# EavnJeong/IEF-VAD

Hardware: AMD Instinct MI355X
Metric: snippets/sec at [B,T=256,d=768] (higher is better)
Workload: dtype f32 emulated: exact 3-term bf16 split of both fp32 operands, 6 bf16 MFMA products, fp32 accumulate

## Files before the change

### ief-vad_amd/csrc/gemm_split.h

```cpp
#pragma once
#include "gemm_bf16.h"

#ifndef GS_EXP_NODMA
#define GS_EXP_NODMA 0
#endif
#ifndef GS_EXP_NOSPLIT
#define GS_EXP_NOSPLIT 0
#endif
#ifndef GS_EXP_NOBAR
#define GS_EXP_NOBAR 0
#endif
#ifndef GS_PN
#define GS_PN 6
#endif
#define GS_BM 128
#define GS_BK 32
#define GS_A_SLOT (GS_BM * 32)
#define GS_BN_OF(NA) ((NA) == 4 ? 256 : 128)
#define GS_LDS_BYTES_OF(NA) ((2 * GS_A_SLOT + 2 * 3 * GS_BN_OF(NA) * 16) * 4)
#define GS_BN GS_BN_OF(4)
#define GS_LDS_BYTES GS_LDS_BYTES_OF(4)

typedef float f32x2 __attribute__((ext_vector_type(2)));
typedef __bf16 bf16x2 __attribute__((ext_vector_type(2)));
typedef unsigned u32x4 __attribute__((ext_vector_type(4)));
typedef _Float16 f16x2 __attribute__((ext_vector_type(2)));
typedef _Float16 f16x8 __attribute__((ext_vector_type(8)));

__device__ __forceinline__ unsigned cvt_pk_bf16(float lo, float hi) {
    return __builtin_bit_cast(unsigned, __builtin_convertvector(f32x2{lo, hi}, bf16x2));
}

struct Split4 {
    f32x4 r;
    __device__ __forceinline__ void plane(unsigned& d0, unsigned& d1, bool peel) {
        d0 = cvt_pk_bf16(r[0], r[1]);
        d1 = cvt_pk_bf16(r[2], r[3]);
        if (peel) {
            r[0] -= __builtin_bit_cast(float, d0 << 16);
            r[1] -= __builtin_bit_cast(float, d0 & 0xffff0000u);
            r[2] -= __builtin_bit_cast(float, d1 << 16);
            r[3] -= __builtin_bit_cast(float, d1 & 0xffff0000u);
        }
    }
    __device__ __forceinline__ void plane_f16(unsigned& d0, unsigned& d1, bool peel) {
        const f16x2 a = __builtin_convertvector(f32x2{r[0], r[1]}, f16x2), b = __builtin_convertvector(f32x2{r[2], r[3]}, f16x2);
        d0 = __builtin_bit_cast(unsigned, a);
        d1 = __builtin_bit_cast(unsigned, b);
        if (peel) {
            const f32x2 fa = __builtin_convertvector(a, f32x2), fb = __builtin_convertvector(b, f32x2);
            r[0] -= fa[0]; r[1] -= fa[1]; r[2] -= fb[0]; r[3] -= fb[1];
        }
    }
};

__global__ __launch_bounds__(256) void iefvad_split_planes_kernel(const float* __restrict__ src, bf16_t* __restrict__ planes, size_t n) {
    const size_t stride = (size_t)gridDim.x * blockDim.x * 4;
    for (size_t i = ((size_t)blockIdx.x * blockDim.x + threadIdx.x) * 4; i < n; i += stride) {
        Split4 s;
        s.r = *(const f32x4*)(src + i);
#pragma unroll
        for (int p = 0; p < 3; ++p) {
            unsigned d0, d1;
            s.plane(d0, d1, p < 2);
            *(uint2*)(planes + (size_t)p * n + i) = make_uint2(d0, d1);
        }
    }
}

#define SPLIT_MANY_MAX 32
struct SplitManyArgs {
    const float* src[SPLIT_MANY_MAX];
    bf16_t* dst[SPLIT_MANY_MAX];
    unsigned n[SPLIT_MANY_MAX];
    int rows[SPLIT_MANY_MAX];
    int count;
};
__global__ __launch_bounds__(256) void iefvad_split_planes_many_kernel(SplitManyArgs a) {
    const int z = blockIdx.y;
    const float* __restrict__ src = a.src[z];
    bf16_t* __restrict__ planes = a.dst[z];
    const size_t n = a.n[z];
    const int n_out = a.rows[z];
    if (n_out == 0) {
// ... 220 lines not shown
                _Pragma("unroll") for (int p = 0; p < NP; ++p) wn[p] = *(const u32x4*)(Wv + p * W_PLANE + ((B) + 1) * 16 * 16); \
                if (GS_NAREAD(B) == 1) vn0 = a_half((B) + 1);                                                   \
                if (GS_NAREAD(B) == 2) { vn0 = a_half((B) + 1); vn1 = a_half((B) + 2); }                        \
            }                                                                                                   \
            if constexpr (!F16) {                                                                               \
                mfma_row(B, NP - 1, w[0]);                                                           \
                mfma_row(B, 0, w[NP - 1]);                                                           \
                mfma_row(B, 1, w[1]);                                                                \
            }                                                                                                   \
            mfma_row(B, 1, w[0]);                                                                    \
            mfma_row(B, 0, w[1]);                                                                    \
            mfma_row(B, 0, w[0]);                                                                    \
            if (!GS_EXP_NOSPLIT) {                                                                              \
                if (GS_NSPLIT(B) >= 1) split_half(B, v0);                                                       \
                if (GS_NSPLIT(B) == 2) split_half((B) + 1, v1);                                                 \
            }                                                                                                   \
            if ((B) == 7) {                                                                                     \
                _Pragma("unroll") for (int a = 0; a < NA; ++a)                                                  \
                    _Pragma("unroll") for (int p = 0; p < NP; ++p) ap[a][p] = an[a][p];                         \
            }                                                                                                   \
            _Pragma("unroll") for (int d = 0; d < GS_NDMA(B); ++d) dma(GS_NDMA(B) * (B) + d);                   \
            if (GS_NREAD(B) > 0) __builtin_amdgcn_sched_group_barrier(0x100, GS_NREAD(B) > 0 ? GS_NREAD(B) : 1, 0); \
            GS_SLOT(B, 0) GS_SLOT(B, 1) GS_SLOT(B, 2) GS_SLOT(B, 3) GS_SLOT(B, 4) GS_SLOT(B, 5)                 \
            GS_SLOT(B, 6) GS_SLOT(B, 7) GS_SLOT(B, 8) GS_SLOT(B, 9) GS_SLOT(B, 10) GS_SLOT(B, 11)               \
            GS_SLOT(B, 12) GS_SLOT(B, 13) GS_SLOT(B, 14) GS_SLOT(B, 15) GS_SLOT(B, 16) GS_SLOT(B, 17)           \
            GS_SLOT(B, 18) GS_SLOT(B, 19) GS_SLOT(B, 20) GS_SLOT(B, 21) GS_SLOT(B, 22) GS_SLOT(B, 23)           \
            GS_FENCE();                                                                                         \
            if ((B) < 7) {                                                                                      \
                _Pragma("unroll") for (int p = 0; p < NP; ++p) w[p] = wn[p];                                    \
                if (GS_NAREAD(B) >= 1) v0 = vn0;                                                                \
                if (GS_NAREAD(B) == 2) v1 = vn1;                                                                \
            }                                                                                                   \
        }
        GS_STEP(0) GS_STEP(1) GS_STEP(2) GS_STEP(3) GS_STEP(4) GS_STEP(5) GS_STEP(6) GS_STEP(7)
#undef GS_STEP
#undef GS_SLOT
#undef GS_VSLOT
#undef GS_NVALU
#undef GS_NDMA
#undef GS_NREAD
#undef GS_NAREAD
#undef GS_NSPLIT
        GS_DIAG_STAMP(0)
        asm volatile("s_waitcnt vmcnt(0)" ::: "memory");
        asm volatile("s_waitcnt lgkmcnt(0)" ::: "memory");
        GS_DIAG_STAMP(1)
        if (!GS_EXP_NOBAR) GB2_BARRIER();
        GS_DIAG_STAMP(2)
    }
#ifdef GB2_CLOCK_DIAG
    if (threadIdx.x == 0 && P.C2) {
        unsigned long long* dg = (unsigned long long*)P.C2 + 2 * (blockIdx.x + gridDim.x * blockIdx.z);
        dg[0] = __builtin_amdgcn_s_memtime() - dg_c0;
        dg[1] = __builtin_amdgcn_s_memrealtime() - dg_r0;
        unsigned long long* dx = (unsigned long long*)P.C2 + 2 * gridDim.x * gridDim.z + 3 * (blockIdx.x + gridDim.x * blockIdx.z);
        dx[0] = dg_acc[0]; dx[1] = dg_acc[1]; dx[2] = dg_acc[2];
    }
    const unsigned long long dg_loop_end = __builtin_amdgcn_s_memtime();
#endif
#undef GS_PIPE
#undef GS_FENCE
#undef GLDS16
    f32x16 unused[NA / 2][4];
    gemm_wave_epilogue<true, NA / 2, !F16>(args, P, smem, m0, n0, wrow0, wcol0, unused, acc16, cscale, F16 ? P.amaxC : nullptr);
#ifdef GB2_CLOCK_DIAG
    if (threadIdx.x == 0 && P.C2) {
        unsigned long long* dy = (unsigned long long*)P.C2 + 5 * gridDim.x * gridDim.z + 2 * (blockIdx.x + gridDim.x * blockIdx.z);
        dy[0] = dg_c0 - dg_entry;
        dy[1] = __builtin_amdgcn_s_memtime() - dg_loop_end;
    }
#endif
}

__global__ __launch_bounds__(256, 1) void iefvad_gemm_split_kernel(GemmBArgs args) {
    extern __shared__ __attribute__((aligned(16))) float smem[];
    gemm_split_body<4>(args, smem);
}

__global__ __launch_bounds__(256, 2) void iefvad_gemm_split_n128_kernel(GemmBArgs args) {
    extern __shared__ __attribute__((aligned(16))) float smem[];
    gemm_split_body<2>(args, smem);
}

__global__ __launch_bounds__(256, 2) void iefvad_gemm_split_f16_n128_kernel(GemmBArgs args) {
    extern __shared__ __attribute__((aligned(16))) float smem[];
    gemm_split_body<2, true>(args, smem);
}

#ifdef GS_EXPERIMENT_F16
__global__ __launch_bounds__(256, 1) void iefvad_gemm_split_f16_kernel(GemmBArgs args) {
    extern __shared__ __attribute__((aligned(16))) float smem[];
    gemm_split_body<4, true>(args, smem);
}
#endif

__global__ __launch_bounds__(256) void iefvad_split_planes_f16_kernel(const float* __restrict__ src, _Float16* __restrict__ planes,
                                                                      size_t n, const float* __restrict__ amax) {
    const float scale = __builtin_ldexpf(1.0f, 13 - amax_exponent(amax_read(amax)));
    const size_t stride = (size_t)gridDim.x * blockDim.x * 4;
    for (size_t i = ((size_t)blockIdx.x * blockDim.x + threadIdx.x) * 4; i < n; i += stride) {
        Split4 s;
        s.r = *(const f32x4*)(src + i) * scale;
#pragma unroll
        for (int p = 0; p < 2; ++p) {
            unsigned d0, d1;
            s.plane_f16(d0, d1, p < 1);
            *(uint2*)(planes + (size_t)p * n + i) = make_uint2(d0, d1);
        }
    }
}
```

### ief-vad_amd/csrc/iefvad.hip

```cpp
#include "../../include/iefvad.h"

#include <hip/hip_runtime.h>
#include <math.h>
#include <stdarg.h>
#include <stdio.h>
#include <stdlib.h>
#include <string.h>

#include <algorithm>
#include <exception>
#include <new>
#include <thread>
#include <vector>

#include "attention_f32.h"
#include "attention_bf16.h"
#include "attention_pbf16.h"
#include "attention_split.h"
#include "common.h"
#include "gather.h"
#include "gemm_f32.h"
#include "gemm_bf16.h"
#include "gemm_split.h"
#include "rowops.h"
// ... 131 lines not shown
            return fail("%s: kernels are built for D=768, T=256, H=8, or D=512, T=256, H=8 in the f32 arithmetic (got D=%d T=%d H=%d)", who,
                        cfg->embed_dim, cfg->seq_len, cfg->num_heads);
        return fail("iefvad_create: kernels are built for D=768, T=256, H=8 (got D=%d T=%d H=%d)",
                    cfg->embed_dim, cfg->seq_len, cfg->num_heads);
    }
    if (cfg->num_layers < 1 || cfg->num_layers > IEFVAD_MAX_LAYERS)
        return fail("%s: num_layers %d outside 1..%d", who, cfg->num_layers, IEFVAD_MAX_LAYERS);
    if (cfg->num_steps < 0 || cfg->num_steps > IEFVAD_MAX_STEPS)
        return fail("%s: num_steps %d outside 0..%d", who, cfg->num_steps, IEFVAD_MAX_STEPS);
    if (cfg->noise_model != IEFVAD_NOISE_GAUSSIAN && cfg->noise_model != IEFVAD_NOISE_STUDENT_T)
        return fail("Unsupported noise_model. Choose 'Gaussian' or 'StudentT'.");
    if (cfg->compute != IEFVAD_COMPUTE_F32 && cfg->compute != IEFVAD_COMPUTE_BF16 && cfg->compute != IEFVAD_COMPUTE_BF16X6 &&
        cfg->compute != IEFVAD_COMPUTE_FP16X3)
        return fail("%s: unknown compute mode %d", who, cfg->compute);
    if (cfg->noise_model == IEFVAD_NOISE_STUDENT_T && !(cfg->nu != 0.f))
        return fail("%s: nu must be non-zero for StudentT", who);
    int ndev = 0;
    HIP_TRY(hipGetDeviceCount(&ndev));
    if (ndev <= 0) return fail("%s: no HIP device", who);
    iefvad_handle* h = new (std::nothrow) iefvad_handle();
    if (!h) return fail("%s: out of host memory", who);
    memset(h, 0, sizeof(*h));
    h->cfg = *cfg;
    h->D = d512 ? IEF_D512 : IEF_D;
    h->DH = h->D / IEF_H;
    {
        const char* v = getenv("IEFVAD_ROWBLOCK_OFF");
        const int off = v ? atoi(v) : 0;
        h->no_inproj_chain = off & 1; h->no_ln_fusion = off & 2; h->no_heads_fusion = off & 4; h->no_chain = off & 8;
    }
    { const char* v = getenv("IEFVAD_ROWBLOCK_MIN_WGS"); h->rowblock_min_wgs = (v && atoi(v) > 0) ? atoi(v) : 128; }
    { const char* v = getenv("IEFVAD_CHAIN_MIN_BLOCKS"); h->chain_min_blocks = (v && atoi(v) > 0) ? atoi(v) : 4; }
    { const char* v = getenv("IEFVAD_PERSIST"); h->persist = !(v && v[0] == '0'); }
    { const char* v = getenv("IEFVAD_DENSE_ENCODER"); h->dense_encoder = v && v[0] == '1'; }
    { const char* v = getenv("IEFVAD_TRAIN_ATTN"); h->train_attn_unfused = v && v[0] == 'u'; }
    { const char* v = getenv("IEFVAD_HOSTPIPE_TRACE"); h->hostpipe_trace = v && v[0] == '1'; }
    hipError_t e = hipGetDevice(&h->device);
    if (e == hipSuccess)
        e = hipFuncSetAttribute((const void*)iefvad_gemm_bf16_kernel, hipFuncAttributeMaxDynamicSharedMemorySize,
                                GB2_LDS_BYTES);
    if (e == hipSuccess)
        e = hipFuncSetAttribute((const void*)iefvad_gemm_bf16_pipe_kernel, hipFuncAttributeMaxDynamicSharedMemorySize,
                                GB2_LDS_BYTES);
    if (e == hipSuccess)
        e = hipFuncSetAttribute((const void*)iefvad_gemm_bf16_w256_kernel, hipFuncAttributeMaxDynamicSharedMemorySize,
                                GB3_LDS_BYTES);
    if (e == hipSuccess)
        e = hipFuncSetAttribute((const void*)iefvad_refine_chain_bf16_kernel, hipFuncAttributeMaxDynamicSharedMemorySize,
                                RC_LDS_BYTES);
    if (e == hipSuccess)
        e = hipFuncSetAttribute((const void*)iefvad_outproj_ln_chain_bf16_kernel, hipFuncAttributeMaxDynamicSharedMemorySize,
                                OC_LDS_BYTES);
    if (e == hipSuccess)
        e = hipFuncSetAttribute((const void*)iefvad_outproj_ln_pchain_bf16_kernel<true, true>, hipFuncAttributeMaxDynamicSharedMemorySize,
                                OP_LDS_BYTES);
    if (e == hipSuccess)
        e = hipFuncSetAttribute((const void*)iefvad_outproj_ln_pchain_bf16_kernel<true, false>, hipFuncAttributeMaxDynamicSharedMemorySize,
                                OP_LDS_BYTES);
    if (e == hipSuccess)
        e = hipFuncSetAttribute((const void*)iefvad_outproj_ln_pchain_bf16_kernel<false, true>, hipFuncAttributeMaxDynamicSharedMemorySize,
                                OP_LDS_BYTES);
    if (e == hipSuccess)
        e = hipFuncSetAttribute((const void*)iefvad_heads_pchain_bf16_kernel, hipFuncAttributeMaxDynamicSharedMemorySize,
                                HP_LDS_BYTES);
    if (e == hipSuccess)
        e = hipFuncSetAttribute((const void*)iefvad_gemm_split_tn256_kernel, hipFuncAttributeMaxDynamicSharedMemorySize, TN_LDS_BYTES_OF(4));
    if (e == hipSuccess)
        e = hipFuncSetAttribute((const void*)iefvad_attention_pbf16_kernel, hipFuncAttributeMaxDynamicSharedMemorySize, APB_LDS_BYTES);
    if (e == hipSuccess)
        e = hipFuncSetAttribute((const void*)iefvad_attention_pbf16_rows_kernel, hipFuncAttributeMaxDynamicSharedMemorySize, APB_LDS_BYTES);
    if (e == hipSuccess) {
        hipDeviceProp_t prop;
        e = hipGetDeviceProperties(&prop, h->device);
        h->num_cus = e == hipSuccess ? prop.multiProcessorCount : 256;
        g_num_cus = h->num_cus;
    }
    if (e == hipSuccess)
        e = hipFuncSetAttribute((const void*)iefvad_gemm_f32_t256_kernel, hipFuncAttributeMaxDynamicSharedMemorySize,
                                GB2_LDS_BYTES);
    if (e == hipSuccess)
        e = hipFuncSetAttribute((const void*)iefvad_gemm_split_n128_kernel, hipFuncAttributeMaxDynamicSharedMemorySize,
                                GS_LDS_BYTES_OF(2));
    if (e == hipSuccess)
        e = hipFuncSetAttribute((const void*)iefvad_attention_split_kernel, hipFuncAttributeMaxDynamicSharedMemorySize,
                                ATS_LDS_BYTES);
    if (e == hipSuccess)
        e = hipFuncSetAttribute((const void*)iefvad_attention_split_rows_kernel, hipFuncAttributeMaxDynamicSharedMemorySize,
                                ATS_LDS_BYTES);
    if (e == hipSuccess)
        e = hipFuncSetAttribute((const void*)iefvad_attention_split_train_kernel, hipFuncAttributeMaxDynamicSharedMemorySize,
                                ATS_LDS_BYTES);
    if (e == hipSuccess)
        e = hipFuncSetAttribute((const void*)iefvad_attention_split_ds_kernel, hipFuncAttributeMaxDynamicSharedMemorySize,
                                ATS_LDS_BYTES);
    if (e == hipSuccess)
        e = hipFuncSetAttribute((const void*)iefvad_attention_split_train_mask_kernel, hipFuncAttributeMaxDynamicSharedMemorySize,
                                ATS_LDS_BYTES);
    if (e == hipSuccess)
        e = hipFuncSetAttribute((const void*)iefvad_heads_chain_bf16_kernel, hipFuncAttributeMaxDynamicSharedMemorySize,
                                HC_LDS_BYTES);
    if (e == hipSuccess)
        e = hipFuncSetAttribute((const void*)iefvad_inproj_chain_bf16_kernel, hipFuncAttributeMaxDynamicSharedMemorySize,
                                IC_LDS_BYTES);
    if (e == hipSuccess)
        e = hipFuncSetAttribute((const void*)iefvad_inproj_chain_f32in_kernel, hipFuncAttributeMaxDynamicSharedMemorySize,
                                IC_LDS_BYTES);
    if (e == hipSuccess)
        e = hipFuncSetAttribute((const void*)iefvad_attention_split_f16_kernel, hipFuncAttributeMaxDynamicSharedMemorySize,
                                ATS_LDS_BYTES);
    if (e == hipSuccess)
        e = hipFuncSetAttribute((const void*)iefvad_gemm_split_f16_n128_kernel, hipFuncAttributeMaxDynamicSharedMemorySize,
                                GS_LDS_BYTES_OF(2));
    if (e == hipSuccess && cfg->compute == IEFVAD_COMPUTE_FP16X3) e = hipMalloc((void**)&h->amax_dev, amax_words(cfg->num_layers, cfg->num_steps, micro_batch(h)) * sizeof(float));
    if (e != hipSuccess) {
        delete h;
        return fail("%s: %s", who, hipGetErrorString(e));
    }
    *out = h;
    return 0;
}

extern "C" int iefvad_create(const iefvad_config* cfg, iefvad_handle** out) { return create_impl("iefvad_create", false, cfg, out); }

extern "C" int iefvad_create_ex(const iefvad_config* cfg, iefvad_handle** out) { return create_impl("iefvad_create_ex", true, cfg, out); }

static void release_events(iefvad_handle* h);
static void release_graphs(iefvad_handle* h);
static void release_meta(iefvad_handle* h);
static void release_train(iefvad_handle* h);
static void release_hostpipe(iefvad_handle* h);

extern "C" void iefvad_destroy(iefvad_handle* h) {
    if (!h) return;
    if (h->arena) (void)hipFree(h->arena);
    if (h->arena_b) (void)hipFree(h->arena_b);
    if (h->chain_stream) (void)hipFree(h->chain_stream);
    if (h->heads_stream) (void)hipFree(h->heads_stream);
    for (int m = 0; m < 2; ++m)
        for (int l = 0; l < IEFVAD_MAX_LAYERS; ++l) {
            if (h->oproj_stream[m][l]) (void)hipFree(h->oproj_stream[m][l]);
            if (h->iproj_stream[m][l]) (void)hipFree(h->iproj_stream[m][l]);
        }
    if (h->arena_s) (void)hipFree(h->arena_s);
    if (h->arena_st) (void)hipFree(h->arena_st);
    if (h->zero_bias) (void)hipFree(h->zero_bias);
    if (h->arena_h) (void)hipFree(h->arena_h);
    if (h->amax_dev) (void)hipFree(h->amax_dev);
    release_events(h);
    release_graphs(h);
    release_meta(h);
    release_train(h);
    release_hostpipe(h);
    delete h;
}

template <typename T>
static int launch_cast(const void* in0, const void* in1, float* o0, float* o1, bf16_t* b0, bf16_t* b1, size_t n, int nsrc,
                       hipStream_t stream) {
    size_t blocks = (n / 4 + 255) / 256;
    if (blocks > 4096) blocks = 4096;
    hipLaunchKernelGGL(iefvad_cast_kernel<T>, dim3((unsigned)blocks, nsrc), dim3(256), 0, stream, (const T*)in0,
                       (const T*)in1, o0, o1, b0, b1, n);
    HIP_TRY(hipGetLastError());
    return 0;
}

// ... 323 lines not shown
    }
}

static const int kF32TinyMaxBlocks64 = 320;
static const int kF32T256MinBlocks = 1536;
static const int kF32SmallMaxBlocks128 = 1024;

static int launch_gemm(const GemmArgs& a, int nz, hipStream_t stream, Timer& tm, int stage) {
    if (a.M % GEMM_BM || a.N % GEMM_BN || a.K % GEMM_BK)
        return fail("gemm: shape M=%d N=%d K=%d not a multiple of the %dx%dx%d tile", a.M, a.N, a.K, GEMM_BM, GEMM_BN,
                    GEMM_BK);
    const int blocks128 = (a.M / GEMM_BM) * (a.N / GEMM_BN) * nz;
    const int blocks64 = (a.M / GEMS_BM) * (a.N / GEMS_BN) * nz;
    const bool t256_ok = (a.N % GB2_BN == 0) && (a.K % 16 == 0) && (a.K >= 32);
    const int blocks256 = t256_ok ? (a.M / GB2_BM) * (a.N / GB2_BN) * nz : 0;
    const bool tiny = blocks64 < kF32TinyMaxBlocks64 && a.K % 64 == 0;
    hipEvent_t e = tm.begin(stage);
    if (tiny) {
        dim3 grid((a.M / GEMT_BM) * (a.N / GEMT_BN), 1, nz);
        hipLaunchKernelGGL(iefvad_gemm_f32_tiny_kernel, grid, dim3(256), 0, stream, a);
    } else if (blocks256 >= kF32T256MinBlocks) {
        GemmBArgs b;
        memset(&b, 0, sizeof(b));
        b.M = a.M; b.N = a.N; b.K = a.K; b.lda = a.lda; b.ldc = a.ldc; b.epi = a.epi; b.alpha = a.alpha; b.qcols = a.qcols;
        for (int m = 0; m < nz; ++m) {
            b.p[m].A = (const bf16_t*)a.p[m].A; b.p[m].W = (const bf16_t*)a.p[m].W;
            b.p[m].bias = a.p[m].bias; b.p[m].C = a.p[m].C; b.p[m].R = a.p[m].R; b.p[m].C2 = a.p[m].C2;
        }
        dim3 grid((a.M / GB2_BM) * (a.N / GB2_BN), 1, nz);
        hipLaunchKernelGGL(iefvad_gemm_f32_t256_kernel, grid, dim3(256), GB2_LDS_BYTES, stream, b);
    } else if (blocks128 < kF32SmallMaxBlocks128) {
        dim3 grid((a.M / GEMS_BM) * (a.N / GEMS_BN), 1, nz);
        hipLaunchKernelGGL(iefvad_gemm_f32_small_kernel, grid, dim3(256), 0, stream, a);
    } else {
        dim3 grid((a.M / GEMM_BM) * (a.N / GEMM_BN), 1, nz);
        hipLaunchKernelGGL(iefvad_gemm_f32_kernel, grid, dim3(256), 0, stream, a);
    }
    tm.end(e);
    tm.gemm_launches += 1;
    HIP_TRY(hipGetLastError());
    return 0;
}

static int launch_gemm_b(const GemmBArgs& a, int nz, hipStream_t stream, Timer& tm, int stage) {
    hipEvent_t e;
    if (a.N % GB2_BN == 0 && a.M % GB2_BM == 0 && a.K % GB2_BK == 0 && a.K >= 2 * GB2_BK) {
        e = tm.begin(stage);
        if (a.M % GB3_BM == 0 && a.epi != EPI_REFINE && (a.M / GB3_BM) * (a.N / GB2_BN) * nz >= 256) {
            dim3 grid((a.M / GB3_BM) * (a.N / GB2_BN), 1, nz);
            hipLaunchKernelGGL(iefvad_gemm_bf16_w256_kernel, grid, dim3(512), GB3_LDS_BYTES, stream, a);
        } else {
            dim3 grid((a.M / GB2_BM) * (a.N / GB2_BN), 1, nz);
            hipLaunchKernelGGL(iefvad_gemm_bf16_pipe_kernel, grid, dim3(256), GB2_LDS_BYTES, stream, a);
        }
    } else {
        if (a.M % GEMM_BM || a.N % GEMM_BN || a.K % GEMMB_BK)
            return fail("gemm(bf16): shape M=%d N=%d K=%d not a multiple of the %dx%dx%d tile", a.M, a.N, a.K, GEMM_BM,
                        GEMM_BN, GEMMB_BK);
        dim3 grid((a.M / GEMM_BM) * (a.N / GEMM_BN), 1, nz);
        e = tm.begin(stage);
        hipLaunchKernelGGL(iefvad_gemm_bf16_v1_kernel, grid, dim3(256), 0, stream, a);
    }
    tm.end(e);
    tm.gemm_launches += 1;
    HIP_TRY(hipGetLastError());
    return 0;
}

static const int kSplitBN = GS_BN_OF(2);
static const int kSplitMinWgs = 72;
static bool split_eligible(int M, int N, int K, int nz) {
    return M % GS_BM == 0 && N % kSplitBN == 0 && K % 64 == 0 && K >= 64 && (M / GS_BM) * (N / kSplitBN) * nz >= kSplitMinWgs;
}

static int launch_gemm_split(const GemmBArgs& a, int nz, hipStream_t stream, Timer& tm, int stage, bool f16 = false) {
    if (a.M % GS_BM || a.N % kSplitBN || a.K % 64 || a.K < 64)
        return fail("gemm(bf16x6): shape M=%d N=%d K=%d not a multiple of the %dx%dx64 tile", a.M, a.N, a.K, GS_BM, kSplitBN);
    if (a.epi == EPI_BIAS_RELU_DOT && (f16 || nz != 1 || !a.p[0].R || !a.p[0].C2))
        return fail("gemm(bf16x6): the dot-product epilogue takes one bf16x6 problem with its vector (R) and its partial sums (C2)");
    dim3 grid((a.M / GS_BM) * (a.N / kSplitBN), 1, nz);
    hipEvent_t e = tm.begin(stage);
    if (f16) hipLaunchKernelGGL(iefvad_gemm_split_f16_n128_kernel, grid, dim3(256), GS_LDS_BYTES_OF(2), stream, a);
    else hipLaunchKernelGGL(iefvad_gemm_split_n128_kernel, grid, dim3(256), GS_LDS_BYTES_OF(2), stream, a);
    tm.end(e);
    tm.gemm_launches += 1;
    HIP_TRY(hipGetLastError());
    return 0;
}

static size_t in_elem_bytes(int in_dtype) { return in_dtype == IEFVAD_IN_F32 ? 4 : 2; }

struct Proj {
    const float* A32[2];
    const bf16_t* A16[2];
    const float* W32[2];
    const bf16_t* W16[2];
    const bf16_t* Ws[2];
    const _Float16* Wh[2];
    const float* amaxW[2];
    const float* amaxA[2];
    float* amaxC[2];
    const float* bias[2];
    float* C[2];
    bf16_t* Cb[2];
    const float* R[2];
    float* C2[2];
    int N, ldc, epi, nz;
    float alpha;
    int qcols;
};

static int launch_proj(const Proj& p, int compute, bool use_split, int D, int rows, hipStream_t stream, Timer& tm, int stage) {
    const bool bf16 = (compute == IEFVAD_COMPUTE_BF16);
    if (p.epi == EPI_BIAS_RELU_DOT && !(use_split && compute == IEFVAD_COMPUTE_BF16X6))
        return fail("gemm: the dot-product epilogue exists in the bf16x6 split kernel only");
    if (use_split) {
        const bool f16 = (compute == IEFVAD_COMPUTE_FP16X3);
        GemmBArgs g;
        memset(&g, 0, sizeof(g));
        g.M = rows; g.N = p.N; g.K = IEF_D; g.lda = IEF_D; g.ldc = p.ldc; g.epi = p.epi; g.alpha = p.alpha; g.qcols = p.qcols;
        g.wplane = p.N * IEF_D * 2;
        for (int m = 0; m < p.nz; ++m) {
            g.p[m].A = (const bf16_t*)p.A32[m];
            g.p[m].W = f16 ? (const bf16_t*)p.Wh[m] : p.Ws[m];
            g.p[m].bias = p.bias[m]; g.p[m].C = p.C[m]; g.p[m].R = p.R[m]; g.p[m].C2 = p.C2[m];
            if (f16) {
                if (!p.amaxA[m] || !p.amaxW[m]) return fail("gemm(fp16x3): missing running-max word");
                g.p[m].amaxA = p.amaxA[m]; g.p[m].amaxW = p.amaxW[m]; g.p[m].amaxC = p.amaxC[m];
            }
        }
        return launch_gemm_split(g, p.nz, stream, tm, stage, f16);
    }
    if (!bf16) {
        GemmArgs g;
        memset(&g, 0, sizeof(g));
        g.M = rows; g.N = p.N; g.K = D; g.lda = D; g.ldc = p.ldc; g.epi = p.epi; g.alpha = p.alpha; g.qcols = p.qcols;
        for (int m = 0; m < p.nz; ++m) {
            g.p[m].A = p.A32[m]; g.p[m].W = p.W32[m]; g.p[m].bias = p.bias[m]; g.p[m].C = p.C[m]; g.p[m].R = p.R[m];
            g.p[m].C2 = p.C2[m];
        }
        return launch_gemm(g, p.nz, stream, tm, stage);
    }
    GemmBArgs g;
    memset(&g, 0, sizeof(g));
    g.M = rows; g.N = p.N; g.K = IEF_D; g.lda = IEF_D; g.ldc = p.ldc; g.epi = p.epi; g.alpha = p.alpha; g.qcols = p.qcols;
    for (int m = 0; m < p.nz; ++m) {
        g.p[m].A = p.A16[m]; g.p[m].W = p.W16[m]; g.p[m].bias = p.bias[m]; g.p[m].C = p.C[m]; g.p[m].Cb = p.Cb[m];
        g.p[m].R = p.R[m]; g.p[m].C2 = p.C2[m];
    }
    return launch_gemm_b(g, p.nz, stream, tm, stage);
}

static int launch_inproj_chain(iefvad_handle* h, int l, const void* const A[2], bool a_fp32, bf16_t* const C[2], int rows, hipStream_t stream, Timer& tm) {
    InProjChainArgs ia;
    memset(&ia, 0, sizeof(ia));
    for (int m = 0; m < 2; ++m) {
        ia.p[m].A = A[m];
        ia.p[m].stream = h->iproj_stream[m][l]; ia.p[m].bias = h->in_b[m][l]; ia.p[m].C = C[m];
    }
    ia.M = rows; ia.alpha = (1.0f / sqrtf((float)IEF_DH)) * 1.4426950408889634f; ia.wave_stride = (unsigned)wstream_wave_stride_bytes(IC_NPASS);
    hipEvent_t e = tm.begin(ST_QKV);
    if (a_fp32) hipLaunchKernelGGL(iefvad_inproj_chain_f32in_kernel, dim3(rows / IC_BM, 2), dim3(512), IC_LDS_BYTES, stream, ia);
    else hipLaunchKernelGGL(iefvad_inproj_chain_bf16_kernel, dim3(rows / IC_BM, 2), dim3(512), IC_LDS_BYTES, stream, ia);
    tm.end(e);
    tm.gemm_launches += 1;
    HIP_TRY(hipGetLastError());
// ... 282 lines not shown
            for (int m = 0; m < 2; ++m) {
                p.A32[m] = att[m]; p.A16[m] = attb[m]; p.W32[m] = h->out_w[m][l]; p.W16[m] = h->out_wb[m][l]; p.Ws[m] = h->out_ws[m][l];
                p.Wh[m] = h->out_wh[m][l]; p.amaxW[m] = h->out_wa[m][l]; p.amaxA[m] = am_att(l, m);
                p.bias[m] = h->out_b[m][l]; p.C[m] = ybuf[m]; p.R[m] = cur[m];
            }
            if (int rc = launch_proj(p, c.compute, splitmb, (int)D, rows, stream, tm, ST_OUT)) return rc;

            LnArgs la;
            memset(&la, 0, sizeof(la));
            la.nrows = rows; la.eps = 1e-5f;
            for (int m = 0; m < 2; ++m) {
                la.x[m] = ybuf[m]; la.g1[m] = h->norm_w[m][l]; la.b1[m] = h->norm_b[m][l];
                if (l == L - 1) { la.g2[m] = h->whiten_w[m]; la.b2[m] = h->whiten_b[m]; }
                la.y[m] = (!bf || l < L - 1) ? xbuf[m] : nullptr;
                la.yb[m] = bf ? xb[m] : nullptr;
                la.amax[m] = am_x(l, m);
            }
            e = tm.begin(ST_LN);
            if (d512) hipLaunchKernelGGL(iefvad_layernorm_kernel<IEF_D512>, dim3((rows + ROW_WAVES - 1) / ROW_WAVES, 2), dim3(256), 0, stream, la);
            else hipLaunchKernelGGL(iefvad_layernorm_kernel<IEF_D>, dim3((rows + ROW_WAVES - 1) / ROW_WAVES, 2), dim3(256), 0, stream, la);
            tm.end(e);
            HIP_TRY(hipGetLastError());
            cur[0] = xbuf[0];
            cur[1] = xbuf[1];
        }

        const float* xt[2] = {xbuf[0], xbuf[1]};
        const bf16_t* xtb[2] = {xb[0], xb[1]};
        bool compacted = false;
        if (rg && !enc_rows_mode && c.compute != IEFVAD_COMPUTE_FP16X3) {
            const int mc = (rg->valid_rows + 255) / 256 * 256;
            if (mc < rows) {
                CompactArgs ca;
                memset(&ca, 0, sizeof(ca));
                for (int m = 0; m < 2; ++m) {
                    if (bf) { ca.xb[m] = xb[m]; ca.xcb[m] = attb[m]; xtb[m] = attb[m]; }
                    else { ca.x[m] = xbuf[m]; ca.xc[m] = att[m]; xt[m] = att[m]; }
                }
                ca.chunks = rg->d_chunks;
                const size_t tail0 = (size_t)rg->valid_rows * D, tailn = (size_t)(mc - rg->valid_rows) * D;
                if (tailn)
                    for (int m = 0; m < 2; ++m)
                        HIP_TRY(bf ? hipMemsetAsync(attb[m] + tail0, 0, tailn * sizeof(bf16_t), stream)
                                   : hipMemsetAsync(att[m] + tail0, 0, tailn * sizeof(float), stream));
                hipEvent_t e = tm.begin(ST_CAST);
                if (d512) hipLaunchKernelGGL(iefvad_compact_rows_kernel<IEF_D512>, dim3(nb, 2), dim3(256), 0, stream, ca);
                else hipLaunchKernelGGL(iefvad_compact_rows_kernel<IEF_D>, dim3(nb, 2), dim3(256), 0, stream, ca);
                tm.end(e);
                HIP_TRY(hipGetLastError());
                rows = mc;
                compacted = true;
            }
        }
        const bool tail_split = splitmb && (!compacted || split_eligible(rows, IEF_D, IEF_D, 1));

        const bool heads_rows = bf && !h->no_heads_fusion && h->heads_stream && rows % HC_BM == 0 && (rows / HC_BM) * HC_THIRDS >= h->rowblock_min_wgs;
        const bool heads_fused = heads_rows;
        const bool chain = bf && K > 0 && !h->no_chain && h->chain_stream && rows % RC_BM == 0 && rows / RC_BM >= h->chain_min_blocks;
        if (heads_rows) {
            HeadsChainArgs ha;
            memset(&ha, 0, sizeof(ha));
            for (int m = 0; m < 2; ++m) ha.A[m] = xtb[m];
            ha.mu[0] = out->image_mu ? mu_i : nullptr;
            ha.lv[0] = out->image_logvar ? lv_i : nullptr;
            ha.mu[1] = out->event_mu ? mu_e : nullptr;
            ha.lv[1] = out->event_logvar ? lv_e : nullptr;
            ha.n[0] = out->w_i ? out->w_i + row0 * D : nullptr;
            ha.n[1] = out->w_e ? out->w_e + row0 * D : nullptr;
            ha.z = z;
            ha.zb = chain ? nullptr : zb;
            const bool means = wim_out || wem_out;
            ha.nsum_part = means ? ybuf[0] : nullptr;
            if (int rc = launch_heads_chain(h, ha, rows, factor, stream, tm)) return rc;
            hipEvent_t e;
            if (means) {
                e = tm.begin(ST_FUSION);
                hipLaunchKernelGGL(iefvad_rowmean_finish_kernel, dim3((2 * rows + 255) / 256), dim3(256), 0, stream, ha.nsum_part,
                                   wim_out, wem_out, rows, HC_NPART);
                tm.end(e);
                HIP_TRY(hipGetLastError());
            }
        }

        if (!heads_fused) {
            Proj p;
            memset(&p, 0, sizeof(p));
            p.N = 2 * (int)D; p.ldc = (int)D; p.epi = EPI_HEADS; p.nz = 2;
            for (int m = 0; m < 2; ++m) {
                p.A32[m] = xt[m]; p.A16[m] = xtb[m]; p.W32[m] = h->head_w[m]; p.W16[m] = h->head_wb[m]; p.Ws[m] = h->head_ws[m]; p.bias[m] = h->head_b[m];
                p.Wh[m] = h->head_wh[m]; p.amaxW[m] = h->head_wa[m]; p.amaxA[m] = am_x(L - 1, m);
            }
            p.C[0] = mu_i; p.C2[0] = lv_i; p.C[1] = mu_e; p.C2[1] = lv_e;
            if (int rc = launch_proj(p, c.compute, tail_split, (int)D, rows, stream, tm, ST_HEAD)) return rc;
        }

        if (!heads_fused) {
            FusionArgs fa;
            memset(&fa, 0, sizeof(fa));
            fa.mu_i = mu_i; fa.lv_i = lv_i; fa.mu_e = mu_e; fa.lv_e = lv_e;
            fa.n_i = out->w_i ? out->w_i + row0 * D : nullptr;
            fa.n_e = out->w_e ? out->w_e + row0 * D : nullptr;
            fa.z = z;
            fa.zb = (bf && !chain) ? zb : nullptr;
            fa.n_i_mean = wim_out;
            fa.n_e_mean = wem_out;
            fa.nrows = rows; fa.factor = factor; fa.eps = c.epsilon;
            fa.z_amax = am_z(0);
            hipEvent_t e = tm.begin(ST_FUSION);
            if (d512) hipLaunchKernelGGL(iefvad_fusion_kernel<IEF_D512>, dim3((rows + ROW_WAVES - 1) / ROW_WAVES), dim3(256), 0, stream, fa);
            else hipLaunchKernelGGL(iefvad_fusion_kernel<IEF_D>, dim3((rows + ROW_WAVES - 1) / ROW_WAVES), dim3(256), 0, stream, fa);
            tm.end(e);
            HIP_TRY(hipGetLastError());
        }

        if (chain)
            if (int rc = launch_refine_chain(h, z, out->fused ? z : nullptr, logits, rows, stream, tm)) return rc;

        const bool fold = tail_split && c.compute == IEFVAD_COMPUTE_BF16X6 && K >= 1;
        float* const fold_part = ybuf[0];
        auto launch_scorer_fold = [&]() -> int {
            hipEvent_t e = tm.begin(ST_SCORER);
            hipLaunchKernelGGL((iefvad_scorer_fold_kernel<IEF_D, IEF_D / kSplitBN>), dim3((rows + ROW_WAVES - 1) / ROW_WAVES), dim3(256), 0,
                               stream, z, h->cls_w, fold_part, h->score_fold, logits, rows);
            tm.end(e);
            HIP_TRY(hipGetLastError());
            return 0;
        };

        for (int k = 0; k < K && !chain; ++k) {
            const bool dot = fold && k == K - 1;
            Proj p;
            memset(&p, 0, sizeof(p));
            p.N = (int)D; p.ldc = (int)D; p.epi = EPI_BIAS_RELU; p.nz = 1;
            p.A32[0] = z; p.A16[0] = zb; p.W32[0] = h->ref_w1[k]; p.W16[0] = h->ref_w1b[k]; p.Ws[0] = h->ref_w1s[k]; p.bias[0] = h->ref_b1[k];
            p.Wh[0] = h->ref_w1h[k]; p.amaxW[0] = h->ref_w1a[k]; p.amaxA[0] = am_z(k); p.amaxC[0] = am_h(k);
            p.C[0] = bf ? nullptr : hbuf; p.Cb[0] = bf ? hb : nullptr;
            if (dot) {
                p.epi = EPI_BIAS_RELU_DOT; p.R[0] = h->score_fold; p.C2[0] = fold_part;
                if (!out->fused) p.C[0] = nullptr;
            }
            if (int rc = launch_proj(p, c.compute, tail_split, (int)D, rows, stream, tm, ST_REFINE)) return rc;
            if (dot) {
                if (int rc = launch_scorer_fold()) return rc;
                if (!out->fused) break;
            }
            memset(&p, 0, sizeof(p));
            p.N = (int)D; p.ldc = (int)D; p.epi = EPI_REFINE; p.alpha = c.lambda_ref; p.nz = 1;
            p.A32[0] = hbuf; p.A16[0] = hb; p.W32[0] = h->ref_w2[k]; p.W16[0] = h->ref_w2b[k]; p.Ws[0] = h->ref_w2s[k]; p.bias[0] = h->ref_b2[k];
            p.Wh[0] = h->ref_w2h[k]; p.amaxW[0] = h->ref_w2a[k]; p.amaxA[0] = am_h(k); p.amaxC[0] = am_z(k + 1);
            p.C[0] = z; p.R[0] = z; p.Cb[0] = (bf && k + 1 < K) ? zb : nullptr;
            if (int rc = launch_proj(p, c.compute, tail_split, (int)D, rows, stream, tm, ST_REFINE)) return rc;
        }

        if (!chain && !fold) {
            hipEvent_t e = tm.begin(ST_SCORER);
            if (d512)
                hipLaunchKernelGGL(iefvad_scorer_kernel<IEF_D512>, dim3((rows + ROW_WAVES - 1) / ROW_WAVES), dim3(256), 0, stream, z,
                                   h->cls_w, h->cls_b, logits, rows);
            else
                hipLaunchKernelGGL(iefvad_scorer_kernel<IEF_D>, dim3((rows + ROW_WAVES - 1) / ROW_WAVES), dim3(256), 0, stream, z,
                                   h->cls_w, h->cls_b, logits, rows);
            tm.end(e);
            HIP_TRY(hipGetLastError());
        }

        if (rg) {
            hipEvent_t e = tm.begin(ST_SCORER);
            if (compacted)
                hipLaunchKernelGGL(iefvad_rows_out_kernel, dim3((rg->valid_rows + 255) / 256), dim3(256), 0, stream, logits, wim_out, wem_out,
                                   rg->logits, rg->w_i_mean, rg->w_e_mean, (const RaggedChunk*)nullptr, rg->valid_rows);
            else
                hipLaunchKernelGGL(iefvad_rows_out_kernel, dim3(nb), dim3(256), 0, stream, logits, wim_out, wem_out, rg->logits,
                                   rg->w_i_mean, rg->w_e_mean, rg->d_chunks, rg->valid_rows);
            tm.end(e);
            HIP_TRY(hipGetLastError());
        }
    }
    return 0;
}
// ... 850 lines not shown
```

Measured before the change: 4.235 million.

## Fuse head projection GEMMs with fusion epilogue in one bf16x6 kernel

Adds a split-bf16x6 GEMM kernel that computes both image and event head projections (mu and logvar columns) per tile and applies the fusion math in the epilogue. It writes z and per-tile row partial sums directly, so the mu/logvar intermediates are never stored or re-read by a separate fusion kernel. The fused path is used only when no per-head outputs are requested, the compute mode is bf16x6 with tail split, and the shape fits. It runs two sequential K passes per tile, which trades some parallelism and longer per-block latency for one fewer launch and less global traffic.

```diff
diff --git a/ief-vad_amd/csrc/gemm_split.h b/ief-vad_amd/csrc/gemm_split.h
--- a/ief-vad_amd/csrc/gemm_split.h
+++ b/ief-vad_amd/csrc/gemm_split.h
@@ -1,5 +1,6 @@
 #pragma once
 #include "gemm_bf16.h"
+#include "heads_fuse_epilogue.h"
 
 #ifndef GS_EXP_NODMA
 #define GS_EXP_NODMA 0
@@ -386,6 +387,201 @@
     gemm_split_body<2>(args, smem);
 }
 
+__device__ __forceinline__ void gemm_split_heads_body(const HeadsFuseArgs& args, float* smem) {
+    constexpr int NA = 2, NP = 3, NT = 6;
+    constexpr int BN = GS_BN_OF(NA);
+    constexpr int W_PLANE = BN * 16;
+    constexpr int W_SLOT = NP * W_PLANE;
+    constexpr int W_BASE = 2 * GS_A_SLOT;
+    constexpr int WROWS = BN / 4;
+    constexpr int NM = NT * NA;
+    const int ntn = args.D / 64;
+    const int bid = xcd_remap(blockIdx.x, gridDim.x);
+    int tm, tn;
+    {
+        const int pn = (GS_PN > 0 && ntn % GS_PN == 0) ? GS_PN : ntn;
+        const int ntm = args.M / GS_BM;
+        const int grp = bid / (ntm * pn), rem = bid - grp * (ntm * pn);
+        tm = rem / pn;
+        tn = grp * pn + (rem - tm * pn);
+    }
+    const int m0 = tm * GS_BM, f0 = tn * 64;
+    const int K = args.K, lda = args.lda;
+    const int wplane = args.wplane;
+
+    const int t = threadIdx.x;
+    const int lane = t & 63, wave = t >> 6;
+    const int wrow0 = wave * 32;
+    const int r16 = lane & 15, q16 = lane >> 4;
+    const int uwave = __builtin_amdgcn_readfirstlane(wave);
+    const int wsrc = uwave * WROWS + (uwave >> 1) * (args.D - 64);
+
+    const int nrecA = (int)((GS_BM - 1) * lda + K) * 4, nrecW = (NP - 1) * wplane + (int)((args.D + 63) * K + K) * 2;
+    const char* const aB[2] = {(const char*)args.A[0] + (size_t)m0 * lda * 4, (const char*)args.A[1] + (size_t)m0 * lda * 4};
+    const char* const wB[2] = {(const char*)args.W[0] + (size_t)f0 * K * 2, (const char*)args.W[1] + (size_t)f0 * K * 2};
+    const auto rsA = __builtin_amdgcn_make_buffer_rsrc((void*)aB[0], 0, nrecA, 0x00020000);
+    const auto rsW = __builtin_amdgcn_make_buffer_rsrc((void*)wB[0], 0, nrecW, 0x00020000);
+    const int arow = lane >> 3, achk = lane & 7;
+    int voA[2];
+#pragma unroll
+    for (int jj = 0; jj < 2; ++jj) voA[jj] = arow * lda * 4 + ((achk ^ (((arow >> 1) & 1) | (jj << 2))) << 4);
+    const int wrow = lane >> 2, wchk = lane & 3;
+    const int voW = wrow * K * 2 + ((wchk ^ ((0xD2 >> (2 * ((wrow >> 2) & 3))) & 3)) << 4);
+#define GLDS16(rs, vo, so, lp) \
+    __builtin_amdgcn_raw_ptr_buffer_load_lds(rs, (__attribute__((address_space(3))) void*)(lp), 16, vo, so, 0, 0)
+
+    const int swa = (r16 >> 1) & 5;
+    const int a_lo = (wrow0 + r16) * 32 + (((2 * q16) ^ swa) << 2);
+    const int a_hi = (wrow0 + r16) * 32 + (((2 * q16 + 1) ^ swa) << 2);
+    const int b_of = r16 * 16 + ((q16 ^ ((0xD2 >> (2 * ((r16 >> 2) & 3))) & 3)) << 2);
+
+    f32x4 acc_i[NA][8], acc_e[NA][8];
+#pragma unroll
+    for (int a = 0; a < NA; ++a)
+#pragma unroll
+        for (int b = 0; b < 8; ++b) acc_i[a][b] = acc_e[a][b] = f32x4{0.f, 0.f, 0.f, 0.f};
+
+    u32x4 ap[NA][NP], an[NA][NP];
+    auto split_half = [&](int hf, const f32x4& v) {
+        Split4 sp;
+        sp.r = v;
+#pragma unroll
+        for (int p = 0; p < NP; ++p) {
+            unsigned d0, d1;
+            sp.plane(d0, d1, p < NP - 1);
+            an[hf >> 1][p][2 * (hf & 1)] = d0;
+            an[hf >> 1][p][2 * (hf & 1) + 1] = d1;
+        }
+    };
+#define GS_FENCE() __builtin_amdgcn_sched_barrier(0)
+#define GS_PIPE(mask) __builtin_amdgcn_sched_group_barrier(mask, 1, 0)
+
+    const int nk = K / GS_BK;
+    {
+        float* Ad0 = smem + uwave * 32 * 32;
+#pragma unroll
+        for (int s = 0; s < 2; ++s)
+#pragma unroll
+            for (int j = 0; j < 4; ++j)
+                GLDS16(rsA, voA[j & 1], ((uwave * 32 + j * 8) * lda + s * GS_BK) * 4, Ad0 + s * GS_A_SLOT + j * 8 * 32);
+        float* Wd0 = smem + W_BASE + uwave * WROWS * 16;
+#pragma unroll
+        for (int p = 0; p < NP; ++p)
+#pragma unroll
+            for (int j = 0; j < WROWS / 16; ++j)
+                GLDS16(rsW, voW, p * wplane + (wsrc + j * 16) * K * 2, Wd0 + p * W_PLANE + j * 16 * 16);
+    }
+    asm volatile("s_waitcnt vmcnt(0)" ::: "memory");
+    GB2_BARRIER();
+#pragma unroll
+    for (int hf = 0; hf < 2 * NA; ++hf)
+        split_half(hf, *(const f32x4*)(smem + (hf >> 1) * 16 * 32 + ((hf & 1) ? a_hi : a_lo)));
+#pragma unroll
+    for (int a = 0; a < NA; ++a)
+#pragma unroll
+        for (int p = 0; p < NP; ++p) ap[a][p] = an[a][p];
+
+    auto k_pass = [&](const int pass, f32x4 (&acc)[NA][8]) __attribute__((always_inline)) {
+        auto mfma_row = [&](int b, int pa, const u32x4& wv) {
+#pragma unroll
+            for (int a = 0; a < NA; ++a)
+                acc[a][b] = __builtin_amdgcn_mfma_f32_16x16x32_bf16(__builtin_bit_cast(bf16x8, ap[a][pa]),
+                                                                   __builtin_bit_cast(bf16x8, wv), acc[a][b], 0, 0, 0);
+        };
+        for (int kt = 0; kt < nk; ++kt) {
+            const bool wself = kt + 1 < nk, aself = kt + 2 < nk;
+            const auto rW = __builtin_amdgcn_make_buffer_rsrc((void*)(wself ? wB[pass] : wB[1]), 0,
+                                                              (wself || pass == 0) ? nrecW : 0, 0x00020000);
+            const auto rA = __builtin_amdgcn_make_buffer_rsrc((void*)(aself ? aB[pass] : aB[1]), 0,
+                                                              (aself || pass == 0) ? nrecA : 0, 0x00020000);
+            float* Wd = smem + W_BASE + ((kt + 1) & 1) * W_SLOT + uwave * WROWS * 16;
+            float* Ad = smem + (kt & 1) * GS_A_SLOT + uwave * 32 * 32;
+            const int kW = (wself ? kt + 1 : 0) * GS_BK * 2, kA = (aself ? kt + 2 : kt + 2 - nk) * GS_BK * 4;
+            auto dma = [&](int d) {
+                if (d < 4) {
+                    GLDS16(rA, voA[d & 1], (uwave * 32 + d * 8) * lda * 4 + kA, Ad + d * 8 * 32);
+                } else {
+                    const int p = (d - 4) / (WROWS / 16), j = (d - 4) % (WROWS / 16);
+                    GLDS16(rW, voW, p * wplane + (wsrc + j * 16) * K * 2 + kW, Wd + p * W_PLANE + j * 16 * 16);
+                }
+            };
+            const float* Wv = smem + W_BASE + (kt & 1) * W_SLOT + b_of;
+            const float* Av = smem + ((kt + 1) & 1) * GS_A_SLOT;
+            auto a_half = [&](int hf) { return *(const f32x4*)(Av + (hf >> 1) * 16 * 32 + ((hf & 1) ? a_hi : a_lo)); };
+            u32x4 w[NP];
+            f32x4 v0 = {0.f, 0.f, 0.f, 0.f};
+#pragma unroll
+            for (int p = 0; p < NP; ++p) w[p] = *(const u32x4*)(Wv + p * W_PLANE);
+            v0 = a_half(0);
+            GS_FENCE();
+#define GSH_NSPLIT(B) ((B) < 4 ? 1 : 0)
+#define GSH_NAREAD(B) ((B) < 7 ? GSH_NSPLIT((B) + 1) : 0)
+#define GSH_NREAD(B) (((B) < 7 ? NP : 0) + GSH_NAREAD(B))
+#define GSH_NDMA(B) ((B) < 5 ? 2 : 0)
+#define GSH_NVALU(B) ((B) == 7 ? 4 * NP * NA : 22 * GSH_NSPLIT(B))
+#define GSH_VSLOT(B, g) (((g) + 1) * GSH_NVALU(B) / NM - (g) * GSH_NVALU(B) / NM)
+#define GSH_SLOT(B, g)                                                                                          \
+            {                                                                                                   \
+                GS_PIPE(0x008);                                                                                 \
+                if (GSH_VSLOT(B, g) > 0) __builtin_amdgcn_sched_group_barrier(0x002, GSH_VSLOT(B, g) > 0 ? GSH_VSLOT(B, g) : 1, 0); \
+                if (GSH_NDMA(B) > 0 && (g) % (NM / 4) == 2 && (g) / (NM / 4) < GSH_NDMA(B)) GS_PIPE(0x020);     \
+            }
+#define GSH_STEP(B)                                                                                             \
+            {                                                                                                   \
+                u32x4 wn[NP];                                                                                   \
+                f32x4 vn0 = {0.f, 0.f, 0.f, 0.f};                                                               \
+                if ((B) < 7) {                                                                                  \
+                    _Pragma("unroll") for (int p = 0; p < NP; ++p) wn[p] = *(const u32x4*)(Wv + p * W_PLANE + ((B) + 1) * 16 * 16); \
+                    if (GSH_NAREAD(B) == 1) vn0 = a_half((B) + 1);                                              \
+                }                                                                                               \
+                mfma_row(B, NP - 1, w[0]);                                                           \
+                mfma_row(B, 0, w[NP - 1]);                                                           \
+                mfma_row(B, 1, w[1]);                                                                \
+                mfma_row(B, 1, w[0]);                                                                \
+                mfma_row(B, 0, w[1]);                                                                \
+                mfma_row(B, 0, w[0]);                                                                \
+                if (GSH_NSPLIT(B) >= 1) split_half(B, v0);                                                      \
+                if ((B) == 7) {                                                                                 \
+                    _Pragma("unroll") for (int a = 0; a < NA; ++a)                                              \
+                        _Pragma("unroll") for (int p = 0; p < NP; ++p) ap[a][p] = an[a][p];                     \
+                }                                                                                               \
+                _Pragma("unroll") for (int d = 0; d < GSH_NDMA(B); ++d) dma(GSH_NDMA(B) * (B) + d);             \
+                if (GSH_NREAD(B) > 0) __builtin_amdgcn_sched_group_barrier(0x100, GSH_NREAD(B) > 0 ? GSH_NREAD(B) : 1, 0); \
+                GSH_SLOT(B, 0) GSH_SLOT(B, 1) GSH_SLOT(B, 2) GSH_SLOT(B, 3) GSH_SLOT(B, 4) GSH_SLOT(B, 5)       \
+                GSH_SLOT(B, 6) GSH_SLOT(B, 7) GSH_SLOT(B, 8) GSH_SLOT(B, 9) GSH_SLOT(B, 10) GSH_SLOT(B, 11)     \
+                GS_FENCE();                                                                                     \
+                if ((B) < 7) {                                                                                  \
+                    _Pragma("unroll") for (int p = 0; p < NP; ++p) w[p] = wn[p];                                \
+                    if (GSH_NAREAD(B) >= 1) v0 = vn0;                                                           \
+                }                                                                                               \
+            }
+            GSH_STEP(0) GSH_STEP(1) GSH_STEP(2) GSH_STEP(3) GSH_STEP(4) GSH_STEP(5) GSH_STEP(6) GSH_STEP(7)
+#undef GSH_STEP
+#undef GSH_SLOT
+#undef GSH_VSLOT
+#undef GSH_NVALU
+#undef GSH_NDMA
+#undef GSH_NREAD
+#undef GSH_NAREAD
+#undef GSH_NSPLIT
+            asm volatile("s_waitcnt vmcnt(0)" ::: "memory");
+            asm volatile("s_waitcnt lgkmcnt(0)" ::: "memory");
+            GB2_BARRIER();
+        }
+    };
+    k_pass(0, acc_i);
+    k_pass(1, acc_e);
+#undef GS_PIPE
+#undef GS_FENCE
+#undef GLDS16
+    heads_fuse_epilogue(args, smem, m0, tn, wrow0, acc_i, acc_e);
+}
+
+__global__ __launch_bounds__(256, 2) void iefvad_gemm_split_heads_fuse_kernel(HeadsFuseArgs args) {
+    extern __shared__ __attribute__((aligned(16))) float smem[];
+    gemm_split_heads_body(args, smem);
+}
+
 __global__ __launch_bounds__(256, 2) void iefvad_gemm_split_f16_n128_kernel(GemmBArgs args) {
     extern __shared__ __attribute__((aligned(16))) float smem[];
     gemm_split_body<2, true>(args, smem);
diff --git a/ief-vad_amd/csrc/heads_fuse_epilogue.h b/ief-vad_amd/csrc/heads_fuse_epilogue.h
--- /dev/null
+++ b/ief-vad_amd/csrc/heads_fuse_epilogue.h
@@ -0,0 +1,67 @@
+#pragma once
+#include "gemm_bf16.h"
+#include "rowops.h"
+
+struct HeadsFuseArgs {
+    const float* A[2];
+    const bf16_t* W[2];
+    const float* bias[2];
+    float* z;
+    float* part;
+    int M, D, K, lda;
+    int wplane;
+    float factor, eps;
+};
+
+__device__ __forceinline__ void heads_fuse_epilogue(const HeadsFuseArgs& args, float* smem, int m0, int tn, int wrow0,
+                                                    f32x4 (&ai)[2][8], f32x4 (&ae)[2][8]) {
+    const int lane = threadIdx.x & 63, wave = threadIdx.x >> 6;
+    const int r16 = lane & 15, q16 = lane >> 4;
+    const int rq = lane >> 4, cq = lane & 15;
+    const int D = args.D, ntile = D / 64;
+    const int col = tn * 64 + 4 * cq;
+    float* E = smem + wave * (32 * GB2_EPI_LD);
+    const f32x4 bmi = *(const f32x4*)(args.bias[0] + col), bli = *(const f32x4*)(args.bias[0] + D + col);
+    const f32x4 bme = *(const f32x4*)(args.bias[1] + col), ble = *(const f32x4*)(args.bias[1] + D + col);
+#pragma unroll
+    for (int x = 0; x < 2; ++x) {
+#pragma unroll
+        for (int b = 0; b < 8; ++b)
+#pragma unroll
+            for (int r = 0; r < 4; ++r) {
+                E[(4 * q16 + r) * GB2_EPI_LD + b * 16 + r16] = ai[x][b][r];
+                E[(16 + 4 * q16 + r) * GB2_EPI_LD + b * 16 + r16] = ae[x][b][r];
+            }
+#pragma unroll
+        for (int u = 0; u < 4; ++u) {
+            const int lr = rq + 4 * u;
+            const int row = m0 + wrow0 + x * 16 + lr;
+            const f32x4 mi = *(const f32x4*)(E + lr * GB2_EPI_LD + 4 * cq) + bmi;
+            const f32x4 li = *(const f32x4*)(E + lr * GB2_EPI_LD + 64 + 4 * cq) + bli;
+            const f32x4 me = *(const f32x4*)(E + (16 + lr) * GB2_EPI_LD + 4 * cq) + bme;
+            const f32x4 le = *(const f32x4*)(E + (16 + lr) * GB2_EPI_LD + 64 + 4 * cq) + ble;
+            f32x4 z;
+            float si = 0.f, se = 0.f;
+#pragma unroll
+            for (int e = 0; e < 4; ++e) {
+                float nie, nee, ze;
+                fuse_elem(mi[e], li[e], me[e], le[e], args.factor, args.eps, nie, nee, ze);
+                z[e] = ze;
+                si += nie;
+                se += nee;
+            }
+            GB2_STORE((f32x4*)(args.z + (size_t)row * D + col), z);
+            if (args.part) {
+                si += dpp_take<0xB1, 0xF>(si, si);  se += dpp_take<0xB1, 0xF>(se, se);
+                si += dpp_take<0x4E, 0xF>(si, si);  se += dpp_take<0x4E, 0xF>(se, se);
+                si += dpp_take<0x141, 0xF>(si, si); se += dpp_take<0x141, 0xF>(se, se);
+                si += dpp_take<0x140, 0xF>(si, si); se += dpp_take<0x140, 0xF>(se, se);
+                if (cq == 0) {
+                    float* pp = args.part + (size_t)row * 2 * ntile + tn;
+                    pp[0] = si;
+                    pp[ntile] = se;
+                }
+            }
+        }
+    }
+}
diff --git a/ief-vad_amd/csrc/iefvad.hip b/ief-vad_amd/csrc/iefvad.hip
--- a/ief-vad_amd/csrc/iefvad.hip
+++ b/ief-vad_amd/csrc/iefvad.hip
@@ -237,6 +237,9 @@
         e = hipFuncSetAttribute((const void*)iefvad_gemm_split_n128_kernel, hipFuncAttributeMaxDynamicSharedMemorySize,
                                 GS_LDS_BYTES_OF(2));
     if (e == hipSuccess)
+        e = hipFuncSetAttribute((const void*)iefvad_gemm_split_heads_fuse_kernel, hipFuncAttributeMaxDynamicSharedMemorySize,
+                                GS_LDS_BYTES_OF(2));
+    if (e == hipSuccess)
         e = hipFuncSetAttribute((const void*)iefvad_attention_split_kernel, hipFuncAttributeMaxDynamicSharedMemorySize,
                                 ATS_LDS_BYTES);
     if (e == hipSuccess)
@@ -726,6 +729,20 @@
     hipEvent_t e = tm.begin(stage);
     if (f16) hipLaunchKernelGGL(iefvad_gemm_split_f16_n128_kernel, grid, dim3(256), GS_LDS_BYTES_OF(2), stream, a);
     else hipLaunchKernelGGL(iefvad_gemm_split_n128_kernel, grid, dim3(256), GS_LDS_BYTES_OF(2), stream, a);
+    tm.end(e);
+    tm.gemm_launches += 1;
+    HIP_TRY(hipGetLastError());
+    return 0;
+}
+
+static bool heads_fuse_eligible(int M, int D, int K) { return M % GS_BM == 0 && D % 256 == 0 && K % 64 == 0 && K >= 64; }
+
+static int launch_heads_fuse(const HeadsFuseArgs& a, hipStream_t stream, Timer& tm) {
+    if (!heads_fuse_eligible(a.M, a.D, a.K))
+        return fail("heads+fusion(bf16x6): shape M=%d D=%d K=%d not a multiple of the %dx256x64 tile", a.M, a.D, a.K, GS_BM);
+    dim3 grid((a.M / GS_BM) * (a.D / 64));
+    hipEvent_t e = tm.begin(ST_HEAD);
+    hipLaunchKernelGGL(iefvad_gemm_split_heads_fuse_kernel, grid, dim3(256), GS_LDS_BYTES_OF(2), stream, a);
     tm.end(e);
     tm.gemm_launches += 1;
     HIP_TRY(hipGetLastError());
@@ -1174,7 +1191,29 @@
             }
         }
 
-        if (!heads_fused) {
+        const bool heads_fold = !heads_fused && tail_split && c.compute == IEFVAD_COMPUTE_BF16X6 && !d512 &&
+                                heads_fuse_eligible(rows, IEF_D, IEF_D) && !out->image_mu &&
+                                !out->image_logvar && !out->event_mu && !out->event_logvar && !out->w_i && !out->w_e;
+        if (heads_fold) {
+            HeadsFuseArgs ha;
+            memset(&ha, 0, sizeof(ha));
+            for (int m = 0; m < 2; ++m) { ha.A[m] = xt[m]; ha.W[m] = h->head_ws[m]; ha.bias[m] = h->head_b[m]; }
+            const bool means = wim_out || wem_out;
+            ha.z = z;
+            ha.part = means ? ybuf[0] : nullptr;
+            ha.M = rows; ha.D = IEF_D; ha.K = IEF_D; ha.lda = IEF_D; ha.wplane = 2 * IEF_D * IEF_D * 2;
+            ha.factor = factor; ha.eps = c.epsilon;
+            if (int rc = launch_heads_fuse(ha, stream, tm)) return rc;
+            if (means) {
+                hipEvent_t e = tm.begin(ST_FUSION);
+                hipLaunchKernelGGL(iefvad_rowmean_finish_kernel, dim3((2 * rows + 255) / 256), dim3(256), 0, stream, ha.part, wim_out,
+                                   wem_out, rows, IEF_D / 64);
+                tm.end(e);
+                HIP_TRY(hipGetLastError());
+            }
+        }
+
+        if (!heads_fused && !heads_fold) {
             Proj p;
             memset(&p, 0, sizeof(p));
             p.N = 2 * (int)D; p.ldc = (int)D; p.epi = EPI_HEADS; p.nz = 2;
@@ -1186,7 +1225,7 @@
             if (int rc = launch_proj(p, c.compute, tail_split, (int)D, rows, stream, tm, ST_HEAD)) return rc;
         }
 
-        if (!heads_fused) {
+        if (!heads_fused && !heads_fold) {
             FusionArgs fa;
             memset(&fa, 0, sizeof(fa));
             fa.mu_i = mu_i; fa.lv_i = lv_i; fa.mu_e = mu_e; fa.lv_e = lv_e;
```

Measured after the change: 4.287 million (median of 6 runs). +1.2%, better.
